# yudaohai666/Sparse_Matrix_Tuning

Measured on AMD Instinct MI355X. Metric: train tokens/sec + peak GB HBM, LLaMA-3-8B SMT(0.71%) at 1/2/4/8 MI355X, higher is better.
Workload: dtype bf16

## Files before the change

### sparse_matrix_tuning_amd/csrc/attn_kernels.hip

```cpp
#include <hip/hip_runtime.h>
#include <stdarg.h>
#include <stdint.h>
#include <stdio.h>
#include <stdlib.h>

#include <type_traits>
#include <utility>

#include "smt_attention.h"
#include "smt_hip.h"

namespace {

thread_local char g_err[512] = "";

int fail(int code, const char* fmt, ...) {
    va_list ap;
    va_start(ap, fmt);
    vsnprintf(g_err, sizeof(g_err), fmt, ap);
    va_end(ap);
    return code;
}

int check_launch(const char* what) {
    hipError_t e = hipGetLastError();
    if (e != hipSuccess) return fail(-4, "%s: %s", what, hipGetErrorString(e));
    return 0;
}

typedef __bf16 bf16x8_t __attribute__((ext_vector_type(8)));
typedef __bf16 bf16x2_t __attribute__((ext_vector_type(2)));
typedef _Float16 f16x8_t __attribute__((ext_vector_type(8)));
typedef _Float16 f16x2_t __attribute__((ext_vector_type(2)));
typedef float f32x2_t __attribute__((ext_vector_type(2)));
typedef short s16x4_t __attribute__((ext_vector_type(4)));
typedef short s16x8_t __attribute__((ext_vector_type(8)));
typedef float f32x16_t __attribute__((ext_vector_type(16)));
typedef uint32_t u32x4_t __attribute__((ext_vector_type(4)));
typedef __attribute__((address_space(3))) s16x4_t lds_s16x4_t;

constexpr int kD = 128;
constexpr int kRowB = 256;
constexpr float kNegInf = -__builtin_huge_valf();

struct Tns {
    const uint16_t* p;
    int64_t sb, sh, ss;
};

__device__ __forceinline__ uint32_t swz(uint32_t row) { return ((row & 3u) << 2) | ((row >> 2) & 3u); }
__device__ __forceinline__ uint32_t lds_off(uint32_t row, uint32_t byte) { return row * kRowB + (byte ^ (swz(row) << 4)); }

__device__ __forceinline__ bf16x8_t row_frag(const uint8_t* img, uint32_t row, uint32_t byte) {
    return *reinterpret_cast<const bf16x8_t*>(img + lds_off(row, byte));
}

struct TrLane {
    uint32_t krow, feat_byte;
};
__device__ __forceinline__ TrLane tr_lane(int lane) {
    const int gi = lane >> 4, q = (lane >> 2) & 3, p = lane & 3;
    return TrLane{8u * (gi >> 1) + q, 2u * (16u * (gi & 1) + 4u * p)};
}
__device__ __forceinline__ bf16x8_t tr_frag(const uint8_t* img, TrLane tl, uint32_t row0, uint32_t col0) {
    const uint32_t r = row0 + tl.krow, byte = 2u * col0 + tl.feat_byte;
    s16x4_t lo = __builtin_amdgcn_ds_read_tr16_b64_v4i16((lds_s16x4_t*)(img + lds_off(r, byte)));
    s16x4_t hi = __builtin_amdgcn_ds_read_tr16_b64_v4i16((lds_s16x4_t*)(img + lds_off(r + 4, byte)));
    const s16x8_t both = __builtin_shufflevector(lo, hi, 0, 1, 2, 3, 4, 5, 6, 7);
    return __builtin_bit_cast(bf16x8_t, both);
}

template <int F>
__device__ __forceinline__ f32x16_t mfma(bf16x8_t a, bf16x8_t b, f32x16_t c) {
    if constexpr (F == SMT_DTYPE_FP16)
        return __builtin_amdgcn_mfma_f32_32x32x16_f16(__builtin_bit_cast(f16x8_t, a), __builtin_bit_cast(f16x8_t, b), c,
                                                      0, 0, 0);
    else return __builtin_amdgcn_mfma_f32_32x32x16_bf16(a, b, c, 0, 0, 0);
}

constexpr bool kPkFwd = false, kPkDq = true, kPkDkv = true;
template <bool PK>
__device__ __forceinline__ f32x2_t fma2(f32x2_t a, f32x2_t b, f32x2_t c) {
    if (PK) return __builtin_elementwise_fma(a, b, c);
    return f32x2_t{__builtin_fmaf(a.x, b.x, c.x), __builtin_fmaf(a.y, b.y, c.y)};
}
template <bool PK>
__device__ __forceinline__ f32x2_t submul2(f32x2_t a, f32x2_t d, f32x2_t p) {
    if (PK) return (a - d) * p;
    return f32x2_t{(a.x - d.x) * p.x, (a.y - d.y) * p.y};
}
template <bool PK>
__device__ __forceinline__ f32x2_t add2(f32x2_t a, f32x2_t b) {
    if (PK) return a + b;
    return f32x2_t{a.x + b.x, a.y + b.y};
}

template <int F>
__device__ __forceinline__ uint32_t pk16(float a, float b) {
    f32x2_t v = {a, b};
    if constexpr (F == SMT_DTYPE_FP16) return __builtin_bit_cast(uint32_t, __builtin_convertvector(v, f16x2_t));
    else return __builtin_bit_cast(uint32_t, __builtin_convertvector(v, bf16x2_t));
}
template <int F>
__device__ __forceinline__ float lo16(uint32_t w) {
    if constexpr (F == SMT_DTYPE_FP16) return (float)__builtin_bit_cast(_Float16, (uint16_t)(w & 0xffffu));
    else return __uint_as_float(w << 16);
}
template <int F>
__device__ __forceinline__ float hi16(uint32_t w) {
    if constexpr (F == SMT_DTYPE_FP16) return (float)__builtin_bit_cast(_Float16, (uint16_t)(w >> 16));
    else return __uint_as_float(w & 0xffff0000u);
}

__device__ __forceinline__ float other_half_max(float x) {
    auto r = __builtin_amdgcn_permlane32_swap(__float_as_uint(x), __float_as_uint(x), false, false);
    return fmaxf(__uint_as_float(r[0]), __uint_as_float(r[1]));
}
__device__ __forceinline__ float halves_sum(float x) {
    auto r = __builtin_amdgcn_permlane32_swap(__float_as_uint(x), __float_as_uint(x), false, false);
    return __uint_as_float(r[0]) + __uint_as_float(r[1]);
}

template <int F>
__device__ __forceinline__ void pack_b_frags(const float (&p)[16], bf16x8_t& f0, bf16x8_t& f1) {
    uint32_t w[8];
#pragma unroll
    for (int i = 0; i < 8; ++i) w[i] = pk16<F>(p[2 * i], p[2 * i + 1]);
#pragma unroll
    for (int h = 0; h < 2; ++h) {
        auto a = __builtin_amdgcn_permlane32_swap(w[4 * h + 0], w[4 * h + 2], false, false);
        auto b = __builtin_amdgcn_permlane32_swap(w[4 * h + 1], w[4 * h + 3], false, false);
        u32x4_t v = {a[0], b[0], a[1], b[1]};
        if (h == 0) f0 = __builtin_bit_cast(bf16x8_t, v);
        else f1 = __builtin_bit_cast(bf16x8_t, v);
    }
}

__device__ __forceinline__ bf16x8_t frag_or_zero(bool valid, const uint16_t* p) {
    if (valid) return *reinterpret_cast<const bf16x8_t*>(p);
    return __builtin_bit_cast(bf16x8_t, u32x4_t{0u, 0u, 0u, 0u});
}

template <int F>
__device__ __forceinline__ void store_row(uint16_t* row, const f32x16_t (&acc)[4], float s, int hi) {
#pragma unroll
    for (int dt = 0; dt < 4; ++dt)
#pragma unroll
        for (int g = 0; g < 4; ++g) {
            uint2 w;
            w.x = pk16<F>(acc[dt][4 * g] * s, acc[dt][4 * g + 1] * s);
            w.y = pk16<F>(acc[dt][4 * g + 2] * s, acc[dt][4 * g + 3] * s);
            const int d = 32 * dt + 8 * g + 4 * hi;
            *reinterpret_cast<uint2*>(row + d) = w;
        }
}

__device__ __forceinline__ void lane_lds(int lane, int l32, int hi, uint32_t& lo_row, uint32_t& lo_t0, uint32_t& lo_t4) {
    const uint32_t r = (uint32_t)l32;
    lo_row = r * kRowB + ((16u * hi) ^ (swz(r) << 4));
    const TrLane tl = tr_lane(lane);
    lo_t0 = tl.krow * kRowB + (tl.feat_byte ^ (swz(tl.krow) << 4));
    lo_t4 = (tl.krow + 4) * kRowB + (tl.feat_byte ^ (swz(tl.krow + 4) << 4));
}

__device__ __forceinline__ int xcd_logical(int bid, int total) {
    const int q8 = total >> 3, r8 = total & 7, xcd = bid & 7;
    return (xcd < r8 ? xcd * (q8 + 1) : r8 * (q8 + 1) + (xcd - r8) * q8) + (bid >> 3);
}

__device__ __forceinline__ uint32_t opaque(uint32_t v) {
    asm volatile("" : "+v"(v));
    return v;
}
template <int IMG>
__device__ __forceinline__ bf16x8_t rowx(const uint8_t* lds, uint32_t lo, int ks) {
    return *reinterpret_cast<const bf16x8_t*>(lds + IMG + (lo ^ (uint32_t)(ks << 5)));
}
template <int IMG>
__device__ __forceinline__ bf16x8_t trx(const uint8_t* lds, uint32_t t0, uint32_t t4, int kq, int dt) {
    const uint32_t x = (uint32_t)(dt << 6);
    s16x4_t lo = __builtin_amdgcn_ds_read_tr16_b64_v4i16((lds_s16x4_t*)(lds + IMG + 4096 * kq + (t0 ^ x)));
    s16x4_t hi = __builtin_amdgcn_ds_read_tr16_b64_v4i16((lds_s16x4_t*)(lds + IMG + 4096 * kq + (t4 ^ x)));
    const s16x8_t both = __builtin_shufflevector(lo, hi, 0, 1, 2, 3, 4, 5, 6, 7);
    return __builtin_bit_cast(bf16x8_t, both);
}

typedef __attribute__((address_space(3))) uint8_t lds_u8_t;
__device__ __forceinline__ void dma16(__amdgpu_buffer_rsrc_t rsrc, uint32_t lds_base, int voff) {
    uint32_t keep;
    asm volatile("s_mov_b32 %0, m0\n\ts_mov_b32 m0, %3\n\ts_nop 0\n\t"
                 "buffer_load_dwordx4 %1, %2, 0 offen lds\n\ts_mov_b32 m0, %0"
                 : "=&s"(keep) : "v"(voff), "s"(rsrc), "s"(lds_base) : "memory");
}
__device__ __forceinline__ uint32_t lds_addr(const uint8_t* p) { return (uint32_t)(uintptr_t)(const lds_u8_t*)p; }
__device__ __forceinline__ __amdgpu_buffer_rsrc_t uniform_rsrc(const void* base, int64_t bytes) {
    const uint64_t a = (uint64_t)(uintptr_t)base;
    const uint32_t lo = __builtin_amdgcn_readfirstlane((uint32_t)a);
    const uint32_t hi = __builtin_amdgcn_readfirstlane((uint32_t)(a >> 32));
    const int n = __builtin_amdgcn_readfirstlane((int)bytes);
    return __builtin_amdgcn_make_buffer_rsrc((void*)(((uint64_t)hi << 32) | lo), 0, n, 0x00020000);
}
__device__ __forceinline__ void vm_wait_all() { asm volatile("s_waitcnt vmcnt(0)" ::: "memory"); }
__device__ __forceinline__ void vm_wait_all_known() { __builtin_amdgcn_s_waitcnt(0x0F70); }
__device__ __forceinline__ void vm_wait_upto(int n) {
    if (n >= 8) asm volatile("s_waitcnt vmcnt(8)" ::: "memory");
    else if (n >= 6) asm volatile("s_waitcnt vmcnt(6)" ::: "memory");
    else if (n >= 4) asm volatile("s_waitcnt vmcnt(4)" ::: "memory");
    else if (n >= 3) asm volatile("s_waitcnt vmcnt(3)" ::: "memory");
    else if (n >= 2) asm volatile("s_waitcnt vmcnt(2)" ::: "memory");
    else asm volatile("s_waitcnt vmcnt(0)" ::: "memory");
}

__device__ __forceinline__ void dma_rows(__amdgpu_buffer_rsrc_t rsrc, int64_t ss, uint32_t img, int img_row0,
                                         int row0, int pieces, int lane) {
#pragma unroll 4
    for (int i = 0; i < pieces; ++i) {
        const int r = row0 + 4 * i + (lane >> 4);
        const uint32_t ir = (uint32_t)(r - img_row0);
        const uint32_t ch = (uint32_t)(lane & 15) ^ swz(ir);
        const uint32_t base = __builtin_amdgcn_readfirstlane(img + (uint32_t)(r - (lane >> 4) - img_row0) * kRowB);
        dma16(rsrc, base, (int)((int64_t)r * ss * 2 + ch * 16));
    }
}

constexpr int kFwdQW = 32, kFwdWaves = 4, kFwdQB = kFwdQW * kFwdWaves, kKV = 64;
constexpr int kDqWaves = 4, kDqQB = kFwdQW * kDqWaves;
constexpr int kTileB = kKV * kRowB;

__device__ __forceinline__ bool key_bit(uint64_t w, int key) { return (w >> (key & 63)) & 1ull; }

constexpr int kIntMax = 0x7fffffff;
__device__ __forceinline__ int doc_clamp(int v, int lo, int hi) { return min(max(v, lo), hi); }
__device__ __forceinline__ int wave_min(int v) {
#pragma unroll
    for (int o = 32; o >= 1; o >>= 1) v = min(v, __shfl_xor(v, o));
    return __builtin_amdgcn_readfirstlane(v);
}
__device__ __forceinline__ int wave_max(int v) {
#pragma unroll
    for (int o = 32; o >= 1; o >>= 1) v = max(v, __shfl_xor(v, o));
    return __builtin_amdgcn_readfirstlane(v);
}
__device__ __forceinline__ int doc_block_min(const int32_t* ds, int q0, int rows, int S, int lane) {
    int g = kIntMax;
    for (int r = q0 + lane; r < min(q0 + rows, S); r += 64) g = min(g, doc_clamp(ds[r], 0, r));
    return wave_min(g);
}

struct DropArgs {
    const uint64_t* seed;
    uint32_t t;
    float r;
};
__device__ __forceinline__ uint32_t drop_mix(uint32_t x) {
    x ^= x >> 16; x *= 0x21F0AAADu; x ^= x >> 15; x *= 0x735A2D97u; x ^= x >> 15;
    return x;
}
__device__ __forceinline__ uint32_t drop_head_key(uint64_t seed, uint32_t bh) {
    return drop_mix((uint32_t)seed + bh * 0x9E3779B9u) ^ (uint32_t)(seed >> 32);
}
__device__ __forceinline__ uint32_t drop_row_key(uint32_t head_key, uint32_t q) {
    return drop_mix(head_key + q * 0x85EBCA6Bu);
}
constexpr uint32_t kDropKeyMul = 0x9E3779B1u;
__device__ __forceinline__ uint32_t drop_word(uint32_t row_key, uint32_t key_term) { return drop_mix(row_key ^ key_term); }
__device__ __forceinline__ bool drop_keep(uint32_t word, uint32_t key_lo2, uint32_t t) {
    return ((word >> (8u * key_lo2)) & 0xFFu) >= t;
}

struct FwdArgs {
    Tns q, k, v;
    uint16_t* o;
    int64_t o_sb, o_sh, o_ss;
    float* lse;
    int lse_ld;
    const uint64_t* kmask;
    int64_t kmask_ld;
    int B, Hq, Hkv, S;
    float sl2;
    DropArgs drop;
    const int32_t* doc_start;
};

struct PairTask {
    int b, hk, hh, blk[2], n;
};
__device__ __forceinline__ PairTask pair_task(int L, int nblk, int G, int Hkv) {
    const int npair = (nblk + 1) / 2;
    const int per_group = G * npair;
    const int grp = L / per_group;
    const int rem = L - grp * per_group;
    const int p = rem / G;
    PairTask t;
    t.b = grp / Hkv;
    t.hk = grp % Hkv;
    t.hh = rem % G;
    t.blk[0] = nblk - 1 - p;
    t.blk[1] = p;
    t.n = (t.blk[1] == t.blk[0]) ? 1 : 2;
    return t;
}

constexpr float kFwdThr = 8.f;


__device__ __forceinline__ float max3f(float a, float b, float c) {
    float r;
    asm("v_max3_f32 %0, %1, %2, %3" : "=v"(r) : "v"(a), "v"(b), "v"(c));
    return r;
}

template <bool KMASK, int F, bool DROP, bool DOC = false>
struct FwdLean {
    const FwdArgs& a;
    uint8_t* lds;
    __amdgpu_buffer_rsrc_t rk, rv;
    uint32_t lds0;
    const uint64_t* km;
    bf16x8_t qf[8];
    f32x16_t o[4];
    float m_run, l_run;
    int qw, qrow, hi, l32, wave, lane, nt, last;
    uint32_t drop_rk;
    int doc_ds, doc_wmax, doc_t0;
    TrLane tl;

    __device__ __forceinline__ FwdLean(const FwdArgs& a_, uint8_t* lds_) : a(a_), lds(lds_) {}

    __device__ __forceinline__ void issue(int t) {
        const uint32_t slot = lds0 + (uint32_t)((t & 1) * 2 * kTileB);
        dma_rows(rk, a.k.ss, slot, t * kKV, t * kKV + 16 * wave, 4, lane);
        dma_rows(rv, a.v.ss, slot + kTileB, t * kKV, t * kKV + 16 * wave, 4, lane);
    }

    template <int SLOT, bool DIAG_>
    __device__ __forceinline__ void compute(int t, bool DIAG) {
        const uint8_t* K = lds + SLOT * 2 * kTileB;
        const uint8_t* V = K + kTileB;
        const int k0 = t * kKV;
        f32x16_t sc[2];
        bf16x8_t kf[3][2];
#pragma unroll
        for (int p = 0; p < 2; ++p)
#pragma unroll
            for (int j = 0; j < 2; ++j) kf[p][j] = row_frag(K, 32 * j + l32, 32 * p + 16 * hi);
#pragma unroll
        for (int ks = 0; ks < 8; ++ks) {
            if (ks + 2 < 8) {
#pragma unroll
                for (int j = 0; j < 2; ++j) kf[(ks + 2) % 3][j] = row_frag(K, 32 * j + l32, 32 * (ks + 2) + 16 * hi);
            }
            __builtin_amdgcn_sched_barrier(0);
#pragma unroll
            for (int j = 0; j < 2; ++j) sc[j] = mfma<F>(kf[ks % 3][j], qf[ks], ks ? sc[j] : f32x16_t{});
            __builtin_amdgcn_sched_barrier(0);
        }
        bf16x8_t vf[3];
        vf[0] = tr_frag(V, tl, 0, 0);
        vf[1] = tr_frag(V, tl, 16, 0);
// ... 250 lines not shown
        if (KMASK) {
            const uint64_t w = km[k0 >> 6];
            if (~w != 0ull) {
#pragma unroll
                for (int i = 0; i < 32; ++i) {
                    const int key = k0 + 32 * (i >> 4) + (i & 3) + 8 * ((i & 15) >> 2) + 4 * hi;
                    if (!key_bit(w, key)) pr[i] = 0.f;
                }
            }
        }
        if constexpr (DOC) {
            if (k0 < doc_wmax) {
#pragma unroll
                for (int i = 0; i < 32; ++i) {
                    const int key = k0 + 32 * (i >> 4) + (i & 3) + 8 * ((i & 15) >> 2) + 4 * hi;
                    if (key < doc_ds) pr[i] = 0.f;
                }
            }
        }
        if constexpr (DROP) {
            const uint32_t kt0 = ((uint32_t)(k0 >> 2) + (uint32_t)hi) * kDropKeyMul;
#pragma unroll
            for (int w = 0; w < 8; ++w) {
                const uint32_t word = drop_word(drop_rk, kt0 + (uint32_t)(8 * (w >> 2) + 2 * (w & 3)) * kDropKeyMul);
#pragma unroll
                for (int c = 0; c < 4; ++c)
                    dp[w >> 2][4 * (w & 3) + c] = drop_keep(word, c, a.drop.t) ? dp[w >> 2][4 * (w & 3) + c] * a.drop.r : 0.f;
            }
        }
#pragma unroll
        for (int i = 0; i < 32; i += 2) {
            const int j = i >> 4, ii = i & 15;
            const f32x2_t r = submul2<kPkDq>(f32x2_t{dp[j][ii], dp[j][ii + 1]}, dv, f32x2_t{pr[i], pr[i + 1]});
            pr[i] = r.x;
            pr[i + 1] = r.y;
        }
        bf16x8_t sf[4];
        pack_b_frags<F>(*reinterpret_cast<const float(*)[16]>(&pr[0]), sf[0], sf[1]);
        pack_b_frags<F>(*reinterpret_cast<const float(*)[16]>(&pr[16]), sf[2], sf[3]);
        const uint32_t t0 = opaque(lo_t0), t4 = opaque(lo_t4);
#pragma unroll
        for (int dt = 0; dt < 4; ++dt) {
#pragma unroll
            for (int kst = 0; kst < 4; ++kst) dq[dt] = mfma<F>(trx<KI>(lds, t0, t4, kst, dt), sf[kst], dq[dt]);
            __builtin_amdgcn_sched_barrier(0);
        }
    }

    template <int SLOT>
    __device__ __forceinline__ void tile(int t) {
        if (t + 1 < nt) issue(t + 1);
        if (t <= last && (!DOC || t >= doc_t0)) compute<SLOT>(t, t == last);
        vm_wait_all();
        __syncthreads();
    }

    __device__ __forceinline__ void run(int b, int h, int hk, int qb) {
        const int tid = threadIdx.x;
        lane = tid & 63;
        wave = __builtin_amdgcn_readfirstlane(tid >> 6);
        hi = lane >> 5;
        l32 = lane & 31;
        const int q0 = qb * kDqQB;
        qw = q0 + wave * kFwdQW;
        qrow = qw + l32;
        const bool qvalid = qrow < a.S;
        const uint16_t* qp = a.q.p + b * a.q.sb + h * a.q.sh;
        const uint16_t* dop = a.dout.p + b * a.dout.sb + h * a.dout.sh;
        const uint16_t* kp = a.k.p + b * a.k.sb + hk * a.k.sh;
        const uint16_t* vp = a.v.p + b * a.v.sb + hk * a.v.sh;
        km = KMASK ? a.kmask + (int64_t)b * a.kmask_ld : nullptr;
        if constexpr (DROP) drop_rk = drop_row_key(drop_head_key(*a.drop.seed, (uint32_t)(b * a.Hq + h)), (uint32_t)qrow);
#pragma unroll
        for (int ks = 0; ks < 8; ++ks) {
            if (qvalid) {
                qf[ks] = *reinterpret_cast<const bf16x8_t*>(qp + qrow * a.q.ss + 16 * ks + 8 * hi);
                df[ks] = *reinterpret_cast<const bf16x8_t*>(dop + qrow * a.dout.ss + 16 * ks + 8 * hi);
            } else {
                qf[ks] = __builtin_bit_cast(bf16x8_t, u32x4_t{0u, 0u, 0u, 0u});
                df[ks] = qf[ks];
            }
        }
        const int64_t srow = ((int64_t)b * a.Hq + h) * a.lse_ld + (qvalid ? qrow : 0);
        lse = qvalid ? a.lse[srow] : 0.f;
        {
            const uint16_t* op = a.o.p + b * a.o.sb + h * a.o.sh;
            float part = 0.f;
#pragma unroll
            for (int ks = 0; ks < 8; ++ks) {
                const u32x4_t ov = qvalid ? *reinterpret_cast<const u32x4_t*>(op + qrow * a.o.ss + 16 * ks + 8 * hi)
                                          : u32x4_t{0u, 0u, 0u, 0u};
                const u32x4_t dv = __builtin_bit_cast(u32x4_t, df[ks]);
#pragma unroll
                for (int j = 0; j < 4; ++j) {
                    part += lo16<F>(ov[j]) * lo16<F>(dv[j]);
                    part += hi16<F>(ov[j]) * hi16<F>(dv[j]);
                }
            }
            dlt = halves_sum(part);
            if (qvalid && hi == 0) a.delta[srow] = dlt;
        }
        const int kv_end = min(a.S, q0 + kDqQB);
        nt = (kv_end + kKV - 1) / kKV;
        last = min(nt - 1, qw / kKV);
        rk = uniform_rsrc(kp, (int64_t)a.S * a.k.ss * 2);
        rv = uniform_rsrc(vp, (int64_t)a.S * a.v.ss * 2);
        lds0 = lds_addr(lds);
        lane_lds(lane, l32, hi, lo_row, lo_t0, lo_t4);
#pragma unroll
        for (int dt = 0; dt < 4; ++dt)
#pragma unroll
            for (int i = 0; i < 16; ++i) dq[dt][i] = 0.f;
        int t0 = 0;
        if constexpr (DOC) {
            const int32_t* ds = a.doc_start + (int64_t)b * a.S;
            doc_ds = qvalid ? doc_clamp(ds[qrow], 0, qrow) : 0;
            doc_wmax = wave_max(doc_ds);
            doc_t0 = wave_min(qvalid ? doc_ds : kIntMax) / kKV;
            t0 = doc_block_min(ds, q0, kDqQB, a.S, lane) / kKV;
        }
        if (DOC || nt > 0) issue(t0);
        vm_wait_all();
        vm_wait_all_known();
        __syncthreads();
        if (t0 & 1) {
            tile<1>(t0);
            ++t0;
        }
        for (int t = t0; t < nt; t += 2) {
            tile<0>(t);
            if (t + 1 < nt) tile<1>(t + 1);
        }
        if (qvalid) store_row<F>(a.dq + b * a.dq_sb + h * a.dq_sh + (int64_t)qrow * a.dq_ss, dq, a.scale, hi);
    }
};

template <bool KMASK, int F, bool DROP, bool DOC = false>
__global__ __launch_bounds__(64 * kDqWaves, 8 / kDqWaves)
void attn_dq_kernel(DqArgs a) {
    static_assert(!(KMASK && DOC), "no key mask beside documents");
    __shared__ __attribute__((aligned(16))) uint8_t lds[2 * 2 * kTileB];
    const int nqb = (a.S + kDqQB - 1) / kDqQB;
    const int G = a.Hq / a.Hkv;
    const int total = nqb * a.Hq * a.B;
    const int L = xcd_logical(blockIdx.x, total);
    const int per_group = G * nqb;
    const int grp = L / per_group;
    const int rem = L - grp * per_group;
    const int hk = grp % a.Hkv;
    DqLean<KMASK, F, DROP, DOC> dl(a, lds);
    dl.run(grp / a.Hkv, hk * G + rem % G, hk, nqb - 1 - rem / G);
}

constexpr int kKB = 256, kKW = 32, kDkvWaves = kKB / kKW, kSlice = 32;
constexpr int kSliceB = kSlice * kRowB;
constexpr int kSliceBuf = 2 * kSliceB + 256;
constexpr int kVImg = kKB * kRowB;

struct DkvArgs {
    Tns q, k, v, dout;
    uint16_t* dk;
    int64_t dk_sb, dk_sh, dk_ss;
    uint16_t* dv;
    int64_t dv_sb, dv_sh, dv_ss;
    const float* lse;
    const float* delta;
    int lse_ld;
    const uint64_t* kmask;
    int64_t kmask_ld;
    int B, Hq, Hkv, S;
    float sl2, scale;
    DropArgs drop;
    const int32_t* doc_end;
};

constexpr int kDkvLeanRing = 2;
static_assert(kDkvLeanRing >= 2 && kDkvLeanRing * kSliceBuf + kVImg <= 160 * 1024, "dK/dV lean ring");
constexpr int kDropRkOff = kDkvLeanRing * kSliceBuf + kVImg, kDropRkB = kSlice * 4;
static_assert(kDropRkOff + kDkvLeanRing * kDropRkB <= 160 * 1024, "dK/dV row keys");
template <int C>
__device__ __forceinline__ uint32_t quad_bcast(uint32_t v) {
    return (uint32_t)__builtin_amdgcn_update_dpp(0, (int)v, C * 0x55, 0xf, 0xf, true);
}
template <bool KMASK, int F, bool DROP, bool DOC = false>
struct DkvLean {
    const DkvArgs& a;
    uint8_t* lds;
    bf16x8_t kf[8];
    f32x16_t dvt[4], dkt[4];
    int G, lane, wave, hi, l32, k0, kw, key, n_sl, n_it, b, hk, per_slice;
    bool kvalid;
    uint32_t lds0;
    uint32_t lo_row, lo_v, lo_t0, lo_t4;
    uint64_t drop_seed;
    uint32_t drop_kt, drop_klo;
    int doc_de, doc_wmin, doc_wmax;

    __device__ __forceinline__ DkvLean(const DkvArgs& a_, uint8_t* lds_) : a(a_), lds(lds_) {}

    __device__ __forceinline__ void issue(int it) {
        const int hh = it / n_sl, sl = n_sl - 1 - (it - hh * n_sl);
        const int h = hk * G + hh;
        const int s0 = k0 + sl * kSlice;
        const uint32_t buf = lds0 + (uint32_t)((it % kDkvLeanRing) * kSliceBuf);
        if (kDkvWaves == 8) {
            const bool is_q = wave < 4;
            const Tns& src = is_q ? a.q : a.dout;
            const uint16_t* base = src.p + b * src.sb + h * src.sh;
            dma_rows(uniform_rsrc(base, (int64_t)a.S * src.ss * 2), src.ss, buf + (is_q ? 0u : (uint32_t)kSliceB), s0,
                     s0 + 8 * (wave & 3), 2, lane);
        } else {
            const uint16_t* qb = a.q.p + b * a.q.sb + h * a.q.sh;
            const uint16_t* db = a.dout.p + b * a.dout.sb + h * a.dout.sh;
            dma_rows(uniform_rsrc(qb, (int64_t)a.S * a.q.ss * 2), a.q.ss, buf, s0, s0 + 8 * wave, 2, lane);
            dma_rows(uniform_rsrc(db, (int64_t)a.S * a.dout.ss * 2), a.dout.ss, buf + (uint32_t)kSliceB, s0,
                     s0 + 8 * wave, 2, lane);
        }
        if (wave < 2 && lane < 8) {
            const float* row = (wave == 0 ? a.lse : a.delta) + ((int64_t)b * a.Hq + h) * a.lse_ld;
            dma16(uniform_rsrc(row, (int64_t)a.S * 4), __builtin_amdgcn_readfirstlane(buf + 2 * kSliceB + 128 * wave),
                  (s0 + 4 * lane) * 4);
        }
        if constexpr (DROP) {
            if (wave == 2 && lane < kSlice) {
                uint32_t* rkeys = reinterpret_cast<uint32_t*>(lds + kDropRkOff + (it % kDkvLeanRing) * kDropRkB);
                rkeys[lane] = drop_row_key(drop_head_key(drop_seed, (uint32_t)(b * a.Hq + h)), (uint32_t)(s0 + lane));
            }
        }
    }

    __device__ __forceinline__ int slice_s0(int it) const {
        const int sl = n_sl - 1 - it % n_sl;
        const int s0 = k0 + sl * kSlice;
        if (DOC && s0 >= doc_wmax) return -1;
        return (s0 + kSlice - 1 < kw) ? -1 : s0;
    }

    template <int SLOT>
    __device__ __forceinline__ void qk(f32x16_t& s, f32x16_t& dp) {
        constexpr int QI = SLOT * kSliceBuf, DI = QI + kSliceB;
        const uint32_t lr = opaque(lo_row), lv = opaque(lo_v);
        s = mfma<F>(rowx<QI>(lds, lr, 0), kf[0], f32x16_t{});
        dp = mfma<F>(rowx<DI>(lds, lr, 0), rowx<0>(lds, lv, 0), f32x16_t{});
#pragma unroll
        for (int ks = 1; ks < 8; ++ks) {
            s = mfma<F>(rowx<QI>(lds, lr, ks), kf[ks], s);
            dp = mfma<F>(rowx<DI>(lds, lr, ks), rowx<0>(lds, lv, ks), dp);
            if (ks & 1) __builtin_amdgcn_sched_barrier(0);
        }
    }

    template <int SLOT>
    __device__ __forceinline__ void pv(int s0, const f32x16_t& s, const f32x16_t& dp) {
        constexpr int QI = SLOT * kSliceBuf, DI = QI + kSliceB;
        const float* cst = reinterpret_cast<const float*>(lds + QI + 2 * kSliceB);
        float pr[16], dsv[16];
        const f32x2_t sl2v = {a.sl2, a.sl2};
#pragma unroll
        for (int g = 0; g < 4; ++g) {
            const float4 lz = *reinterpret_cast<const float4*>(cst + 8 * g + 4 * hi);
#pragma unroll
            for (int h = 0; h < 2; ++h) {
                const int i = 4 * g + 2 * h;
                const f32x2_t l2 = h ? f32x2_t{lz.z, lz.w} : f32x2_t{lz.x, lz.y};
                const f32x2_t e = fma2<kPkDkv>(f32x2_t{s[i], s[i + 1]}, sl2v, -l2);
                pr[i] = __builtin_amdgcn_exp2f(e.x);
                pr[i + 1] = __builtin_amdgcn_exp2f(e.y);
            }
        }
        if (s0 < kw + kKW - 1) {
#pragma unroll
            for (int i = 0; i < 16; ++i) {
                const int q = s0 + (i & 3) + 8 * (i >> 2) + 4 * hi;
                if (key > q) pr[i] = 0.f;
            }
        }
        if (KMASK && !kvalid) {
#pragma unroll
            for (int i = 0; i < 16; ++i) pr[i] = 0.f;
        }
        if constexpr (DOC) {
            if (s0 + kSlice > doc_wmin) {
#pragma unroll
                for (int i = 0; i < 16; ++i) {
                    const int q = s0 + (i & 3) + 8 * (i >> 2) + 4 * hi;
                    if (q >= doc_de) pr[i] = 0.f;
                }
            }
        }
        bool kp[16];
        if constexpr (DROP) {
            const uint32_t* rkeys = reinterpret_cast<const uint32_t*>(lds + kDropRkOff + SLOT * kDropRkB);
#pragma unroll
            for (int g = 0; g < 4; ++g) {
                const uint32_t wq = drop_word(rkeys[8 * g + 4 * hi + (lane & 3)], drop_kt);
                kp[4 * g + 0] = drop_keep(quad_bcast<0>(wq), drop_klo, a.drop.t);
                kp[4 * g + 1] = drop_keep(quad_bcast<1>(wq), drop_klo, a.drop.t);
                kp[4 * g + 2] = drop_keep(quad_bcast<2>(wq), drop_klo, a.drop.t);
                kp[4 * g + 3] = drop_keep(quad_bcast<3>(wq), drop_klo, a.drop.t);
            }
        }
#pragma unroll
        for (int g = 0; g < 4; ++g) {
            const float4 dz = *reinterpret_cast<const float4*>(cst + 32 + 8 * g + 4 * hi);
#pragma unroll
            for (int h = 0; h < 2; ++h) {
                const int i = 4 * g + 2 * h;
                const f32x2_t d2 = h ? f32x2_t{dz.z, dz.w} : f32x2_t{dz.x, dz.y};
                f32x2_t dpv = {dp[i], dp[i + 1]};
                if constexpr (DROP)
                    dpv = f32x2_t{kp[i] ? dp[i] * a.drop.r : 0.f, kp[i + 1] ? dp[i + 1] * a.drop.r : 0.f};
                const f32x2_t r = submul2<kPkDkv>(dpv, d2, f32x2_t{pr[i], pr[i + 1]});
                dsv[i] = r.x;
                dsv[i + 1] = r.y;
            }
        }
        if constexpr (DROP) {
#pragma unroll
            for (int i = 0; i < 16; ++i) pr[i] = kp[i] ? pr[i] : 0.f;
        }
        bf16x8_t pf[2], sf[2];
        pack_b_frags<F>(pr, pf[0], pf[1]);
        pack_b_frags<F>(dsv, sf[0], sf[1]);
        const uint32_t t0 = opaque(lo_t0), t4 = opaque(lo_t4);
#pragma unroll
        for (int dt = 0; dt < 4; ++dt)
#pragma unroll
            for (int kq = 0; kq < 2; ++kq) {
                dvt[dt] = mfma<F>(trx<DI>(lds, t0, t4, kq, dt), pf[kq], dvt[dt]);
                dkt[dt] = mfma<F>(trx<QI>(lds, t0, t4, kq, dt), sf[kq], dkt[dt]);
                if (kq) __builtin_amdgcn_sched_barrier(0);
            }
    }

    template <int SLOT>
    __device__ __forceinline__ void step(int it) {
        constexpr int R = kDkvLeanRing;
        if (it + R - 1 < n_it) issue(it + R - 1);
        const int s0 = slice_s0(it);
        if (s0 >= 0) {
            f32x16_t s, dp;
            qk<SLOT>(s, dp);
            pv<SLOT>(s0, s, dp);
        }
        vm_wait_upto(per_slice * max(0, min(R - 2, n_it - 2 - it)));
        __syncthreads();
    }

    template <int SLOT>
    __device__ __forceinline__ void steps(int it0) {
        if (it0 + SLOT < n_it) {
            step<SLOT>(it0 + SLOT);
            if constexpr (SLOT + 1 < kDkvLeanRing) steps<SLOT + 1>(it0);
        }
    }

    __device__ __forceinline__ void run(int b_, int hk_, int kb) {
        b = b_;
        hk = hk_;
        G = a.Hq / a.Hkv;
        const int tid = threadIdx.x;
        lane = tid & 63;
        wave = __builtin_amdgcn_readfirstlane(tid >> 6);
        hi = lane >> 5;
        l32 = lane & 31;
        k0 = kb * kKB;
        kw = k0 + wave * kKW;
        key = kw + l32;
        kvalid = !KMASK || (key < a.S && key_bit(a.kmask[(int64_t)b * a.kmask_ld + (key >> 6)], key));
        if constexpr (DROP) {
            drop_seed = *a.drop.seed;
            drop_kt = (uint32_t)(key >> 2) * kDropKeyMul;
            drop_klo = (uint32_t)(key & 3);
        }
        const uint16_t* kp = a.k.p + b * a.k.sb + hk * a.k.sh;
        const uint16_t* vp = a.v.p + b * a.v.sb + hk * a.v.sh;
        lds0 = lds_addr(lds);
        dma_rows(uniform_rsrc(vp, (int64_t)a.S * a.v.ss * 2), a.v.ss, lds0 + kDkvLeanRing * kSliceBuf, k0, kw, kKW / 4, lane);
        lane_lds(lane, l32, hi, lo_row, lo_t0, lo_t4);
        lo_v = lo_row + (uint32_t)(kDkvLeanRing * kSliceBuf + wave * kKW * kRowB);
#pragma unroll
        for (int ks = 0; ks < 8; ++ks) {
            kf[ks] = frag_or_zero(key < a.S, kp + (int64_t)key * a.k.ss + 16 * ks + 8 * hi);
        }
        int s_end = a.S;
        if constexpr (DOC) {
            const int32_t* de = a.doc_end + (int64_t)b * a.S;
            const bool valid = key < a.S;
            doc_de = valid ? doc_clamp(de[key], key + 1, a.S) : kIntMax;
            doc_wmin = wave_min(doc_de);
            doc_wmax = wave_max(valid ? doc_de : 0);
            const int lk = min(k0 + kKB, a.S) - 1;
            s_end = doc_clamp(__builtin_amdgcn_readfirstlane(de[lk]), lk + 1, a.S);
        }
        n_sl = (s_end - k0 + kSlice - 1) / kSlice;
        n_it = G * n_sl;
#pragma unroll
        for (int dt = 0; dt < 4; ++dt)
#pragma unroll
            for (int i = 0; i < 16; ++i) { dvt[dt][i] = 0.f; dkt[dt][i] = 0.f; }
        per_slice = (kDkvWaves == 8 ? 2 : 4) + (wave < 2 ? 1 : 0);
#pragma unroll
        for (int i = 0; i < kDkvLeanRing - 1; ++i)
            if (i < n_it) issue(i);
        vm_wait_all();
        vm_wait_all_known();
        __syncthreads();
        for (int it = 0; it < n_it; it += kDkvLeanRing) steps<0>(it);
        if constexpr (DROP) {
#pragma unroll
            for (int dt = 0; dt < 4; ++dt)
#pragma unroll
                for (int i = 0; i < 16; ++i) dvt[dt][i] *= a.drop.r;
        }
        if (key < a.S) {
            uint16_t* dkr = a.dk + b * a.dk_sb + hk * a.dk_sh + (int64_t)key * a.dk_ss;
            uint16_t* dvr = a.dv + b * a.dv_sb + hk * a.dv_sh + (int64_t)key * a.dv_ss;
#pragma unroll
            for (int dt = 0; dt < 4; ++dt)
#pragma unroll
                for (int g = 0; g < 4; ++g) {
                    const int d = 32 * dt + 8 * g + 4 * hi;
                    uint2 w;
                    w.x = pk16<F>(dkt[dt][4 * g] * a.scale, dkt[dt][4 * g + 1] * a.scale);
                    w.y = pk16<F>(dkt[dt][4 * g + 2] * a.scale, dkt[dt][4 * g + 3] * a.scale);
                    *reinterpret_cast<uint2*>(dkr + d) = w;
                    w.x = pk16<F>(dvt[dt][4 * g], dvt[dt][4 * g + 1]);
                    w.y = pk16<F>(dvt[dt][4 * g + 2], dvt[dt][4 * g + 3]);
                    *reinterpret_cast<uint2*>(dvr + d) = w;
                }
        }
    }
};

template <bool KMASK, int F, bool DROP, bool DOC = false>
__global__ __launch_bounds__(kDkvWaves * 64, 2)
void attn_dkdv_kernel(DkvArgs a) {
    static_assert(!(KMASK && DOC), "no key mask beside documents");
    __shared__ __attribute__((aligned(16))) uint8_t lds[kVImg + kDkvLeanRing * (kSliceBuf + (DROP ? kDropRkB : 0))];
    const int nkb = (a.S + kKB - 1) / kKB;
    const int total = ((nkb + 1) / 2) * a.Hkv * a.B;
    const PairTask t = pair_task(xcd_logical(blockIdx.x, total), nkb, 1, a.Hkv);
#pragma nounroll
    for (int i = 0; i < t.n; ++i) {
        if (i) __syncthreads();
        DkvLean<KMASK, F, DROP, DOC> dl(a, lds);
        dl.run(t.b, t.hk, t.blk[1 - i]);
    }
}

__global__ __launch_bounds__(256)
void attn_dropout_mask_kernel(uint8_t* keep, DropArgs drop, int S, int64_t n_words) {
    const int64_t i = (int64_t)blockIdx.x * 256 + threadIdx.x;
    if (i >= n_words) return;
    const int wpr = (S + 3) >> 2;
    const int64_t row = i / wpr;
    const int kw = (int)(i - row * wpr);
    const uint32_t bh = (uint32_t)(row / S), q = (uint32_t)(row - (int64_t)bh * S);
    const uint32_t word = drop_word(drop_row_key(drop_head_key(*drop.seed, bh), q), (uint32_t)kw * kDropKeyMul);
    for (int c = 0; c < 4; ++c) {
        const int key = 4 * kw + c;
        if (key < S) keep[row * S + key] = drop_keep(word, (uint32_t)c, drop.t) ? 1 : 0;
    }
}

constexpr int kDecCols = 32;
constexpr int kDecPartial = kDecCols * (kD + 2);

struct DecArgs {
    Tns q, k, v;
    uint16_t* o;
    int64_t o_sb, o_sh, o_ss;
    float* lse;
    const uint64_t* kmask;
    int64_t kmask_ld;
    float* ws;
    int Hq, Hkv, G, Sq, q_offset, ncols, ncb, nsplit, tps;
    float sl2;
};
struct DecPosArgs : DecArgs {
    const int64_t* pos;
    int pos_stride, cap;
};

__device__ __forceinline__ float* dec_ws_o(const DecArgs& a, int64_t slot, int col) {
    return a.ws + (slot * kDecCols + col) * kD;
}
__device__ __forceinline__ float* dec_ws_ml(const DecArgs& a, int64_t nslots, int64_t slot, int col) {
    return a.ws + nslots * kDecCols * kD + (slot * kDecCols + col) * 2;
}


__device__ __forceinline__ void dec_load_q(bf16x8_t (&qf)[8], bool cvalid, const uint16_t* qp, int hi) {
#pragma unroll
    for (int ks = 0; ks < 8; ++ks) qf[ks] = frag_or_zero(cvalid, qp + 16 * ks + 8 * hi);
}

__device__ __forceinline__ void dec_zero_unseen_v(uint8_t* V, uint64_t w_any, int lane) {
    if (~w_any == 0ull) return;
    if (!key_bit(w_any, lane)) {
#pragma unroll
        for (int c = 0; c < 16; ++c) *reinterpret_cast<u32x4_t*>(V + lane * kRowB + 16 * c) = u32x4_t{0u, 0u, 0u, 0u};
    }
    __syncthreads();
}

template <int F>
__device__ __forceinline__ void dec_scores(float (&x)[32], const uint8_t* K, const bf16x8_t (&qf)[8], int l32, int hi) {
    f32x16_t sc[2];
#pragma unroll
    for (int ks = 0; ks < 8; ++ks)
#pragma unroll
        for (int j = 0; j < 2; ++j)
            sc[j] = mfma<F>(row_frag(K, 32 * j + l32, 32 * ks + 16 * hi), qf[ks], ks ? sc[j] : f32x16_t{});
#pragma unroll
    for (int j = 0; j < 2; ++j)
#pragma unroll
        for (int i = 0; i < 16; ++i) x[16 * j + i] = sc[j][i];
}

template <int F>
__device__ __forceinline__ void dec_softmax_pv(float (&x)[32], const uint8_t* V, TrLane tl, float sl2, float& m_run,
                                               float& l_run, f32x16_t (&o)[4]) {
    float mx = x[0];
#pragma unroll
    for (int i = 1; i < 32; ++i) mx = fmaxf(mx, x[i]);
    const float m_tile = other_half_max(mx) * sl2;
    const bool move = m_tile > m_run + kFwdThr;
    const float m_new = move ? m_tile : m_run;
    const float alpha = move ? __builtin_amdgcn_exp2f(m_run - m_new) : 1.f;
    const float m_use = (m_new == kNegInf) ? 0.f : m_new;
    float sum = 0.f;
#pragma unroll
    for (int i = 0; i < 32; ++i) {
        x[i] = __builtin_amdgcn_exp2f(__builtin_fmaf(x[i], sl2, -m_use));
        sum += x[i];
    }
    l_run = l_run * alpha + sum;
    m_run = m_new;
    if (__builtin_amdgcn_ballot_w64(move) != 0) {
#pragma unroll
        for (int dt = 0; dt < 4; ++dt)
#pragma unroll
            for (int i = 0; i < 16; ++i) o[dt][i] *= alpha;
    }
    bf16x8_t pf[4];
    pack_b_frags<F>(*reinterpret_cast<const float(*)[16]>(&x[0]), pf[0], pf[1]);
    pack_b_frags<F>(*reinterpret_cast<const float(*)[16]>(&x[16]), pf[2], pf[3]);
#pragma unroll
    for (int n = 0; n < 16; ++n) o[n >> 2] = mfma<F>(tr_frag(V, tl, 16 * (n & 3), 32 * (n >> 2)), pf[n & 3], o[n >> 2]);
}

__device__ __forceinline__ void dec_empty_split(const DecArgs& a, int64_t nslots, int64_t slot, int l32) {
    float* ml = dec_ws_ml(a, nslots, slot, l32);
    ml[0] = kNegInf;
    ml[1] = 0.f;
}

template <int F, bool DIRECT>
__device__ __forceinline__ void dec_finish(const DecArgs& a, const f32x16_t (&o)[4], float m_run, float l_run,
                                           int64_t nslots, int64_t slot, bool cvalid, int l32, int hi, int64_t o_idx,
                                           int64_t lse_idx) {
    const float l_tot = halves_sum(l_run);
    if (!cvalid) return;
    if (DIRECT) {
        store_row<F>(a.o + o_idx, o, l_tot > 0.f ? 1.f / l_tot : 0.f, hi);
        if (a.lse && hi == 0) a.lse[lse_idx] = l_tot > 0.f ? m_run + __log2f(l_tot) : __builtin_huge_valf();
    } else {
        const bool any = l_tot > 0.f;
        if (any) {
            float* po = dec_ws_o(a, slot, l32);
#pragma unroll
            for (int dt = 0; dt < 4; ++dt)
#pragma unroll
                for (int g = 0; g < 4; ++g)
                    *reinterpret_cast<float4*>(po + 32 * dt + 8 * g + 4 * hi) =
                        float4{o[dt][4 * g], o[dt][4 * g + 1], o[dt][4 * g + 2], o[dt][4 * g + 3]};
        }
        if (hi == 0) {
            float* ml = dec_ws_ml(a, nslots, slot, l32);
            ml[0] = any ? m_run : kNegInf;
            ml[1] = any ? l_tot : 0.f;
        }
    }
}

template <bool KMASK, int F, bool DIRECT, class Args>
__global__ __launch_bounds__(64)
void attn_decode_kernel(Args a) {
    constexpr bool POS = std::is_same<Args, DecPosArgs>::value;
    __shared__ __attribute__((aligned(16))) uint8_t lds[2 * 2 * kTileB];
    const int cb = blockIdx.x, sp = blockIdx.y, bh = blockIdx.z;
// ... 830 lines not shown
```

Baseline: 39420.

## Split dK/dV backward into producer and consumer waves with LDS hand-off

Restructures the attention dK/dV backward kernel so that each 32-key block is handled by a pair of waves. A producer wave keeps K and V fragments in registers and computes S, dP, P and dS, then writes the packed P/dS fragments to a double-buffered LDS hand-off area. A consumer wave accumulates dV and dK from that area. The key block shrinks from 256 to 128 keys, the Q/dO ring deepens to 4 slots with a two-slice prefetch, the V LDS image is removed, and packed FP32 math is disabled for this kernel. The goal is to overlap the softmax-gradient elementwise work with the MFMA accumulation and to cut register pressure per wave, at the cost of extra LDS traffic and more barriers.

```diff
diff --git a/sparse_matrix_tuning_amd/csrc/attn_kernels.hip b/sparse_matrix_tuning_amd/csrc/attn_kernels.hip
--- a/sparse_matrix_tuning_amd/csrc/attn_kernels.hip
+++ b/sparse_matrix_tuning_amd/csrc/attn_kernels.hip
@@ -78,7 +78,7 @@
     else return __builtin_amdgcn_mfma_f32_32x32x16_bf16(a, b, c, 0, 0, 0);
 }
 
-constexpr bool kPkFwd = false, kPkDq = true, kPkDkv = true;
+constexpr bool kPkFwd = false, kPkDq = true, kPkDkv = false;
 template <bool PK>
 __device__ __forceinline__ f32x2_t fma2(f32x2_t a, f32x2_t b, f32x2_t c) {
     if (PK) return __builtin_elementwise_fma(a, b, c);
@@ -203,8 +203,10 @@
 __device__ __forceinline__ void vm_wait_all() { asm volatile("s_waitcnt vmcnt(0)" ::: "memory"); }
 __device__ __forceinline__ void vm_wait_all_known() { __builtin_amdgcn_s_waitcnt(0x0F70); }
 __device__ __forceinline__ void vm_wait_upto(int n) {
-    if (n >= 8) asm volatile("s_waitcnt vmcnt(8)" ::: "memory");
+    if (n >= 10) asm volatile("s_waitcnt vmcnt(10)" ::: "memory");
+    else if (n >= 8) asm volatile("s_waitcnt vmcnt(8)" ::: "memory");
     else if (n >= 6) asm volatile("s_waitcnt vmcnt(6)" ::: "memory");
+    else if (n >= 5) asm volatile("s_waitcnt vmcnt(5)" ::: "memory");
     else if (n >= 4) asm volatile("s_waitcnt vmcnt(4)" ::: "memory");
     else if (n >= 3) asm volatile("s_waitcnt vmcnt(3)" ::: "memory");
     else if (n >= 2) asm volatile("s_waitcnt vmcnt(2)" ::: "memory");
@@ -761,10 +763,16 @@
     dl.run(grp / a.Hkv, hk * G + rem % G, hk, nqb - 1 - rem / G);
 }
 
-constexpr int kKB = 256, kKW = 32, kDkvWaves = kKB / kKW, kSlice = 32;
+constexpr int kKB = 128, kKW = 32, kDkvPairs = kKB / kKW, kDkvWaves = 2 * kDkvPairs, kSlice = 32;
 constexpr int kSliceB = kSlice * kRowB;
 constexpr int kSliceBuf = 2 * kSliceB + 256;
-constexpr int kVImg = kKB * kRowB;
+constexpr int kDkvRing = 4, kDkvAhead = kDkvRing - 2;
+static_assert(kDkvAhead >= 1, "dK/dV ring");
+constexpr int kHoFrag = 64 * 16, kHoPair = 4 * kHoFrag, kHoSlot = kDkvPairs * kHoPair;
+constexpr int kHoOff = kDkvRing * kSliceBuf;
+constexpr int kDropRkOff = kHoOff + 2 * kHoSlot, kDropRkB = kSlice * 4;
+static_assert(kDropRkOff + kDkvRing * kDropRkB <= 160 * 1024, "dK/dV LDS");
+static_assert(kHoOff % 16 == 0, "hand-off fragments are 16-byte accesses");
 
 struct DkvArgs {
     Tns q, k, v, dout;
@@ -783,10 +791,6 @@
     const int32_t* doc_end;
 };
 
-constexpr int kDkvLeanRing = 2;
-static_assert(kDkvLeanRing >= 2 && kDkvLeanRing * kSliceBuf + kVImg <= 160 * 1024, "dK/dV lean ring");
-constexpr int kDropRkOff = kDkvLeanRing * kSliceBuf + kVImg, kDropRkB = kSlice * 4;
-static_assert(kDropRkOff + kDkvLeanRing * kDropRkB <= 160 * 1024, "dK/dV row keys");
 template <int C>
 __device__ __forceinline__ uint32_t quad_bcast(uint32_t v) {
     return (uint32_t)__builtin_amdgcn_update_dpp(0, (int)v, C * 0x55, 0xf, 0xf, true);
@@ -795,79 +799,82 @@
 struct DkvLean {
     const DkvArgs& a;
     uint8_t* lds;
-    bf16x8_t kf[8];
+    bf16x8_t kf[8], vf[8];
     f32x16_t dvt[4], dkt[4];
-    int G, lane, wave, hi, l32, k0, kw, key, n_sl, n_it, b, hk, per_slice;
+    int G, lane, wave, pair, hi, l32, k0, kw, key, n_sl, n_it, b, hk, per_slice, c_sl, d_h, d_sl;
     bool kvalid;
     uint32_t lds0;
-    uint32_t lo_row, lo_v, lo_t0, lo_t4;
+    uint32_t lo_row, lo_t0, lo_t4, lo_ho;
     uint64_t drop_seed;
     uint32_t drop_kt, drop_klo;
     int doc_de, doc_wmin, doc_wmax;
 
     __device__ __forceinline__ DkvLean(const DkvArgs& a_, uint8_t* lds_) : a(a_), lds(lds_) {}
 
-    __device__ __forceinline__ void issue(int it) {
-        const int hh = it / n_sl, sl = n_sl - 1 - (it - hh * n_sl);
-        const int h = hk * G + hh;
-        const int s0 = k0 + sl * kSlice;
-        const uint32_t buf = lds0 + (uint32_t)((it % kDkvLeanRing) * kSliceBuf);
-        if (kDkvWaves == 8) {
-            const bool is_q = wave < 4;
-            const Tns& src = is_q ? a.q : a.dout;
-            const uint16_t* base = src.p + b * src.sb + h * src.sh;
-            dma_rows(uniform_rsrc(base, (int64_t)a.S * src.ss * 2), src.ss, buf + (is_q ? 0u : (uint32_t)kSliceB), s0,
-                     s0 + 8 * (wave & 3), 2, lane);
-        } else {
-            const uint16_t* qb = a.q.p + b * a.q.sb + h * a.q.sh;
-            const uint16_t* db = a.dout.p + b * a.dout.sb + h * a.dout.sh;
-            dma_rows(uniform_rsrc(qb, (int64_t)a.S * a.q.ss * 2), a.q.ss, buf, s0, s0 + 8 * wave, 2, lane);
-            dma_rows(uniform_rsrc(db, (int64_t)a.S * a.dout.ss * 2), a.dout.ss, buf + (uint32_t)kSliceB, s0,
-                     s0 + 8 * wave, 2, lane);
-        }
-        if (wave < 2 && lane < 8) {
-            const float* row = (wave == 0 ? a.lse : a.delta) + ((int64_t)b * a.Hq + h) * a.lse_ld;
-            dma16(uniform_rsrc(row, (int64_t)a.S * 4), __builtin_amdgcn_readfirstlane(buf + 2 * kSliceB + 128 * wave),
+    template <int SLOT>
+    __device__ __forceinline__ void issue() {
+        const int h = hk * G + d_h;
+        const int s0 = k0 + d_sl * kSlice;
+        if (--d_sl < 0) { d_sl = n_sl - 1; ++d_h; }
+        const uint32_t buf = lds0 + (uint32_t)(SLOT * kSliceBuf);
+        const uint16_t* qb = a.q.p + b * a.q.sb + h * a.q.sh;
+        const uint16_t* db = a.dout.p + b * a.dout.sb + h * a.dout.sh;
+        dma_rows(uniform_rsrc(qb, (int64_t)a.S * a.q.ss * 2), a.q.ss, buf, s0, s0 + 8 * pair, 2, lane);
+        dma_rows(uniform_rsrc(db, (int64_t)a.S * a.dout.ss * 2), a.dout.ss, buf + (uint32_t)kSliceB, s0, s0 + 8 * pair, 2,
+                 lane);
+        if (pair < 2 && lane < 8) {
+            const float* row = (pair == 0 ? a.lse : a.delta) + ((int64_t)b * a.Hq + h) * a.lse_ld;
+            dma16(uniform_rsrc(row, (int64_t)a.S * 4), __builtin_amdgcn_readfirstlane(buf + 2 * kSliceB + 128 * pair),
                   (s0 + 4 * lane) * 4);
         }
         if constexpr (DROP) {
-            if (wave == 2 && lane < kSlice) {
-                uint32_t* rkeys = reinterpret_cast<uint32_t*>(lds + kDropRkOff + (it % kDkvLeanRing) * kDropRkB);
+            if (pair == 2 && lane < kSlice) {
+                uint32_t* rkeys = reinterpret_cast<uint32_t*>(lds + kDropRkOff + SLOT * kDropRkB);
                 rkeys[lane] = drop_row_key(drop_head_key(drop_seed, (uint32_t)(b * a.Hq + h)), (uint32_t)(s0 + lane));
             }
         }
     }
 
-    __device__ __forceinline__ int slice_s0(int it) const {
-        const int sl = n_sl - 1 - it % n_sl;
-        const int s0 = k0 + sl * kSlice;
+    __device__ __forceinline__ int next_s0() {
+        const int s0 = k0 + c_sl * kSlice;
+        if (--c_sl < 0) c_sl = n_sl - 1;
         if (DOC && s0 >= doc_wmax) return -1;
         return (s0 + kSlice - 1 < kw) ? -1 : s0;
     }
 
     template <int SLOT>
-    __device__ __forceinline__ void qk(f32x16_t& s, f32x16_t& dp) {
+    __device__ __forceinline__ void produce(int it) {
+        const int s0 = next_s0();
+        if (s0 < 0) return;
         constexpr int QI = SLOT * kSliceBuf, DI = QI + kSliceB;
-        const uint32_t lr = opaque(lo_row), lv = opaque(lo_v);
-        s = mfma<F>(rowx<QI>(lds, lr, 0), kf[0], f32x16_t{});
-        dp = mfma<F>(rowx<DI>(lds, lr, 0), rowx<0>(lds, lv, 0), f32x16_t{});
+        const uint32_t lr = opaque(lo_row);
+        const float* cst = reinterpret_cast<const float*>(lds + QI + 2 * kSliceB);
+        bf16x8_t qf[8], df[8];
+        float4 lzv[4], dzv[4];
+#pragma unroll
+        for (int ks = 0; ks < 8; ++ks) {
+            qf[ks] = rowx<QI>(lds, lr, ks);
+            df[ks] = rowx<DI>(lds, lr, ks);
+        }
+#pragma unroll
+        for (int g = 0; g < 4; ++g) {
+            lzv[g] = *reinterpret_cast<const float4*>(cst + 8 * g + 4 * hi);
+            dzv[g] = *reinterpret_cast<const float4*>(cst + 32 + 8 * g + 4 * hi);
+        }
+        __builtin_amdgcn_sched_barrier(0);
+        f32x16_t s = mfma<F>(qf[0], kf[0], f32x16_t{});
+        f32x16_t dp = mfma<F>(df[0], vf[0], f32x16_t{});
 #pragma unroll
         for (int ks = 1; ks < 8; ++ks) {
-            s = mfma<F>(rowx<QI>(lds, lr, ks), kf[ks], s);
-            dp = mfma<F>(rowx<DI>(lds, lr, ks), rowx<0>(lds, lv, ks), dp);
-            if (ks & 1) __builtin_amdgcn_sched_barrier(0);
-        }
-    }
-
-    template <int SLOT>
-    __device__ __forceinline__ void pv(int s0, const f32x16_t& s, const f32x16_t& dp) {
-        constexpr int QI = SLOT * kSliceBuf, DI = QI + kSliceB;
-        const float* cst = reinterpret_cast<const float*>(lds + QI + 2 * kSliceB);
+            s = mfma<F>(qf[ks], kf[ks], s);
+            dp = mfma<F>(df[ks], vf[ks], dp);
+        }
+        __builtin_amdgcn_sched_barrier(0);
         float pr[16], dsv[16];
         const f32x2_t sl2v = {a.sl2, a.sl2};
 #pragma unroll
         for (int g = 0; g < 4; ++g) {
-            const float4 lz = *reinterpret_cast<const float4*>(cst + 8 * g + 4 * hi);
+            const float4 lz = lzv[g];
 #pragma unroll
             for (int h = 0; h < 2; ++h) {
                 const int i = 4 * g + 2 * h;
@@ -911,7 +918,7 @@
         }
 #pragma unroll
         for (int g = 0; g < 4; ++g) {
-            const float4 dz = *reinterpret_cast<const float4*>(cst + 32 + 8 * g + 4 * hi);
+            const float4 dz = dzv[g];
 #pragma unroll
             for (int h = 0; h < 2; ++h) {
                 const int i = 4 * g + 2 * h;
@@ -931,37 +938,74 @@
         bf16x8_t pf[2], sf[2];
         pack_b_frags<F>(pr, pf[0], pf[1]);
         pack_b_frags<F>(dsv, sf[0], sf[1]);
+        bf16x8_t* ho = reinterpret_cast<bf16x8_t*>(lds + kHoOff + (it & 1) * kHoSlot + lo_ho);
+        ho[0 * 64] = pf[0];
+        ho[1 * 64] = pf[1];
+        ho[2 * 64] = sf[0];
+        ho[3 * 64] = sf[1];
+    }
+
+    template <int SLOT>
+    __device__ __forceinline__ void consume(int it) {
+        if (next_s0() < 0) return;
+        constexpr int QI = SLOT * kSliceBuf, DI = QI + kSliceB;
+        const bf16x8_t* ho = reinterpret_cast<const bf16x8_t*>(lds + kHoOff + (it & 1) * kHoSlot + lo_ho);
+        const bf16x8_t pf[2] = {ho[0 * 64], ho[1 * 64]}, sf[2] = {ho[2 * 64], ho[3 * 64]};
         const uint32_t t0 = opaque(lo_t0), t4 = opaque(lo_t4);
+        bf16x8_t dof[4][2], qtf[4][2];
 #pragma unroll
         for (int dt = 0; dt < 4; ++dt)
 #pragma unroll
             for (int kq = 0; kq < 2; ++kq) {
-                dvt[dt] = mfma<F>(trx<DI>(lds, t0, t4, kq, dt), pf[kq], dvt[dt]);
-                dkt[dt] = mfma<F>(trx<QI>(lds, t0, t4, kq, dt), sf[kq], dkt[dt]);
-                if (kq) __builtin_amdgcn_sched_barrier(0);
-            }
+                dof[dt][kq] = trx<DI>(lds, t0, t4, kq, dt);
+                qtf[dt][kq] = trx<QI>(lds, t0, t4, kq, dt);
+            }
+        __builtin_amdgcn_sched_barrier(0);
+#pragma unroll
+        for (int dt = 0; dt < 4; ++dt)
+#pragma unroll
+            for (int kq = 0; kq < 2; ++kq) {
+                dvt[dt] = mfma<F>(dof[dt][kq], pf[kq], dvt[dt]);
+                dkt[dt] = mfma<F>(qtf[dt][kq], sf[kq], dkt[dt]);
+            }
+        __builtin_amdgcn_sched_barrier(0);
+    }
+
+    template <bool CONS, int SLOT>
+    __device__ __forceinline__ void steps(int it0) {
+        constexpr int R = kDkvRing;
+        const int it = it0 + SLOT;
+        if (it <= n_it) {
+            if constexpr (CONS) {
+                if (it + kDkvAhead < n_it) issue<(SLOT + kDkvAhead) % R>();
+                if (it >= 1) consume<(SLOT + R - 1) % R>(it - 1);
+                vm_wait_upto(per_slice * max(0, min(kDkvAhead - 1, n_it - 2 - it)));
+            } else {
+                if (it < n_it) produce<SLOT>(it);
+            }
+            __syncthreads();
+            if constexpr (SLOT + 1 < R) steps<CONS, SLOT + 1>(it0);
+        }
     }
 
     template <int SLOT>
-    __device__ __forceinline__ void step(int it) {
-        constexpr int R = kDkvLeanRing;
-        if (it + R - 1 < n_it) issue(it + R - 1);
-        const int s0 = slice_s0(it);
-        if (s0 >= 0) {
-            f32x16_t s, dp;
-            qk<SLOT>(s, dp);
-            pv<SLOT>(s0, s, dp);
-        }
-        vm_wait_upto(per_slice * max(0, min(R - 2, n_it - 2 - it)));
+    __device__ __forceinline__ void prologue() {
+        if (SLOT < n_it) issue<SLOT>();
+        if constexpr (SLOT + 1 < kDkvAhead) prologue<SLOT + 1>();
+    }
+
+    template <bool CONS>
+    __device__ __forceinline__ void sweep() {
+        c_sl = n_sl - 1;
+        if constexpr (CONS) {
+            d_h = 0;
+            d_sl = n_sl - 1;
+            prologue<0>();
+        }
+        vm_wait_all();
+        vm_wait_all_known();
         __syncthreads();
-    }
-
-    template <int SLOT>
-    __device__ __forceinline__ void steps(int it0) {
-        if (it0 + SLOT < n_it) {
-            step<SLOT>(it0 + SLOT);
-            if constexpr (SLOT + 1 < kDkvLeanRing) steps<SLOT + 1>(it0);
-        }
+        for (int it0 = 0; it0 <= n_it; it0 += kDkvRing) steps<CONS, 0>(it0);
     }
 
     __device__ __forceinline__ void run(int b_, int hk_, int kb) {
@@ -971,27 +1015,15 @@
         const int tid = threadIdx.x;
         lane = tid & 63;
         wave = __builtin_amdgcn_readfirstlane(tid >> 6);
+        pair = wave & (kDkvPairs - 1);
         hi = lane >> 5;
         l32 = lane & 31;
         k0 = kb * kKB;
-        kw = k0 + wave * kKW;
+        kw = k0 + pair * kKW;
         key = kw + l32;
-        kvalid = !KMASK || (key < a.S && key_bit(a.kmask[(int64_t)b * a.kmask_ld + (key >> 6)], key));
-        if constexpr (DROP) {
-            drop_seed = *a.drop.seed;
-            drop_kt = (uint32_t)(key >> 2) * kDropKeyMul;
-            drop_klo = (uint32_t)(key & 3);
-        }
-        const uint16_t* kp = a.k.p + b * a.k.sb + hk * a.k.sh;
-        const uint16_t* vp = a.v.p + b * a.v.sb + hk * a.v.sh;
         lds0 = lds_addr(lds);
-        dma_rows(uniform_rsrc(vp, (int64_t)a.S * a.v.ss * 2), a.v.ss, lds0 + kDkvLeanRing * kSliceBuf, k0, kw, kKW / 4, lane);
         lane_lds(lane, l32, hi, lo_row, lo_t0, lo_t4);
-        lo_v = lo_row + (uint32_t)(kDkvLeanRing * kSliceBuf + wave * kKW * kRowB);
-#pragma unroll
-        for (int ks = 0; ks < 8; ++ks) {
-            kf[ks] = frag_or_zero(key < a.S, kp + (int64_t)key * a.k.ss + 16 * ks + 8 * hi);
-        }
+        lo_ho = (uint32_t)(pair * kHoPair + lane * 16);
         int s_end = a.S;
         if constexpr (DOC) {
             const int32_t* de = a.doc_end + (int64_t)b * a.S;
@@ -1004,18 +1036,29 @@
         }
         n_sl = (s_end - k0 + kSlice - 1) / kSlice;
         n_it = G * n_sl;
+        per_slice = 4 + (pair < 2 ? 1 : 0);
+        if constexpr (DROP) drop_seed = *a.drop.seed;
+        if (wave < kDkvPairs) {
+            kvalid = !KMASK || (key < a.S && key_bit(a.kmask[(int64_t)b * a.kmask_ld + (key >> 6)], key));
+            if constexpr (DROP) {
+                drop_kt = (uint32_t)(key >> 2) * kDropKeyMul;
+                drop_klo = (uint32_t)(key & 3);
+            }
+            const uint16_t* kp = a.k.p + b * a.k.sb + hk * a.k.sh + (int64_t)key * a.k.ss;
+            const uint16_t* vp = a.v.p + b * a.v.sb + hk * a.v.sh + (int64_t)key * a.v.ss;
+#pragma unroll
+            for (int ks = 0; ks < 8; ++ks) {
+                kf[ks] = frag_or_zero(key < a.S, kp + 16 * ks + 8 * hi);
+                vf[ks] = frag_or_zero(key < a.S, vp + 16 * ks + 8 * hi);
+            }
+            sweep<false>();
+            return;
+        }
 #pragma unroll
         for (int dt = 0; dt < 4; ++dt)
 #pragma unroll
             for (int i = 0; i < 16; ++i) { dvt[dt][i] = 0.f; dkt[dt][i] = 0.f; }
-        per_slice = (kDkvWaves == 8 ? 2 : 4) + (wave < 2 ? 1 : 0);
-#pragma unroll
-        for (int i = 0; i < kDkvLeanRing - 1; ++i)
-            if (i < n_it) issue(i);
-        vm_wait_all();
-        vm_wait_all_known();
-        __syncthreads();
-        for (int it = 0; it < n_it; it += kDkvLeanRing) steps<0>(it);
+        sweep<true>();
         if constexpr (DROP) {
 #pragma unroll
             for (int dt = 0; dt < 4; ++dt)
@@ -1046,7 +1089,7 @@
 __global__ __launch_bounds__(kDkvWaves * 64, 2)
 void attn_dkdv_kernel(DkvArgs a) {
     static_assert(!(KMASK && DOC), "no key mask beside documents");
-    __shared__ __attribute__((aligned(16))) uint8_t lds[kVImg + kDkvLeanRing * (kSliceBuf + (DROP ? kDropRkB : 0))];
+    __shared__ __attribute__((aligned(16))) uint8_t lds[kDropRkOff + (DROP ? kDkvRing * kDropRkB : 0)];
     const int nkb = (a.S + kKB - 1) / kKB;
     const int total = ((nkb + 1) / 2) * a.Hkv * a.B;
     const PairTask t = pair_task(xcd_logical(blockIdx.x, total), nkb, 1, a.Hkv);
```

After: 39480, median of 2. About the same (+0.1%).
